# EI-CoreBioinformatics/portcullis

Hardware: AMD Instinct MI355X
Metric: junc_reads_per_sec (higher is better)
Workload: dtype int32; 1 GPU; BASELINE configs[2]: synthetic 199999998 paired-end 150-bp reads, 25 contigs of GRCh38 lengths (3088286401 bp), 249999 junctions, orientation FR; reads_total=199999998, junctions_total=249999, contigs=25, reads_rank0=199999998, pairs_rank0=66692850

## Files before the change

### portcullis_amd/csrc/pjb_api.hip

```cpp
#include "pjb_host.hip.h"
#include "pjb_kernels.hip.h"
#include "pjb_chain.hip.h"
#include "pjb_flight.hip.h"

extern "C" {

namespace {
std::mutex g_host_mu;
std::map<void *, size_t> g_host_registered;
}
void *pjb_host_alloc(size_t bytes) {
    if (bytes >= ((size_t)8 << 20)) {
        const size_t huge = (size_t)2 << 20, len = (bytes + huge - 1) & ~(huge - 1);
        void *p = mmap(nullptr, len, PROT_READ | PROT_WRITE, MAP_PRIVATE | MAP_ANONYMOUS, -1, 0);
        if (p != MAP_FAILED) {
            (void)madvise(p, len, MADV_HUGEPAGE);
            const size_t nt = std::min<size_t>(4, len >> 24);
            auto touch = [&](size_t t) {
                const size_t per = ((len / std::max<size_t>(nt, 1)) + huge - 1) & ~(huge - 1), a = std::min(len, per * t), b = std::min(len, a + per);
                for (size_t o = a; o < b; o += 4096) ((volatile uint8_t *)p)[o] = 0;
            };
            if (nt <= 1) touch(0);
            else {
                std::vector<std::thread> th;
// ... 664 lines not shown
    return PJB_OK;
}

int pjb_reset_kernel_timing(pjb_ctx *c) {
    if (!c) return PJB_ERR_ARG;
    std::fill(c->kcount.begin(), c->kcount.end(), 0);
    std::fill(c->kms.begin(), c->kms.end(), 0.0);
    return PJB_OK;
}

int pjb_set_option(pjb_ctx *c, const char *name, int64_t value) {
    if (!c || !name) return PJB_ERR_ARG;
    if (c->n_fl) return fail(c, PJB_ERR_STATE, "set_option: target %d is still queued", c->fl[0].tid);
    const std::string n = name;
    if (n == "overlap") c->side_stream = value != 0;
    else if (n == "dense_ids") c->dense_ids = value != 0;
    else if (n == "extra_dense") c->extra_dense_only = value != 0;
    else if (n == "sort_floor") c->sort_floor = (u32)std::max<int64_t>(1, std::min<int64_t>(value, 1 << 30));
    else if (n == "window_skip") c->window_skip = value != 0;
    else if (n == "run_sort") c->run_sort = value != 0;
    else if (n == "run_window") {
        if (value < 0 || value > (int64_t)RUN_W) return fail(c, PJB_ERR_ARG, "set_option: run_window takes 0 (the default, %u) to %u", RUN_W, RUN_W);
        c->run_window = (u32)value;
    } else if (n == "pair_range") {
        int shift = -1;
        for (int k = 0; k <= PAIR_RANGE_SHIFT_MAX; k++)
            if (value == (int64_t)1 << k) shift = k;
        if (shift < 0) return fail(c, PJB_ERR_ARG, "set_option: pair_range takes 1, 2, 4, 8, 16 or 32 slices a range (the default: %d)", 1 << PAIR_RANGE_SHIFT_DEFAULT);
        c->pair_range_shift = shift;
    } else if (n == "grow_batch") {
        if (value < 0 || value > 32768) return fail(c, PJB_ERR_ARG, "set_option: grow_batch takes 0 (the default: what the pool holds) to 32768 trees");
        c->model.grow_batch = (u32)value;
    } else if (n == "knn_chunk") {
        if (value < 0 || value > (1 << 22)) return fail(c, PJB_ERR_ARG, "set_option: knn_chunk takes 0 (the default: sized to fill the chip) to %d base rows", 1 << 22);
        c->model.knn_chunk = (u32)value;
    } else if (n == "mem_limit") {
        if (value < 0) return fail(c, PJB_ERR_ARG, "set_option: mem_limit takes 0 (the default: no limit) or a number of bytes");
        std::lock_guard<std::mutex> lk(c->mem.mu);
        c->mem.limit = (size_t)value;
    } else if (n == "list_cap") c->list_cap_forced = (u32)std::max<int64_t>(0, std::min<int64_t>(value, 1 << 30));
    else return fail(c, PJB_ERR_ARG, "set_option: unknown option '%s'", name);
    return PJB_OK;
}

int pjb_memory_info(const pjb_ctx *c, pjb_memory *out) {
    if (!c || !out) return PJB_ERR_ARG;
// ... 39 lines not shown
```

### portcullis_amd/csrc/pjb_chain.hip.h

```cpp
#pragma once

constexpr unsigned K6_BLOCKS = 128;

static size_t rows_upper_bound(const pjb_ctx *c) {
    size_t n = c->rows_n;
    for (int k = 0; k < c->n_fl; k++)
        if (c->fl[k].queued) n += c->fl[k].lim.junc_limit;
    return n;
}

static void wait_flight(pjb_ctx *c, Flight &f) {
    if (f.queued) (void)hipEventSynchronize(c->sl[f.slot].ev_done);
}

static int rows_table_reserve(pjb_ctx *c, Flight &f, u32 JL) {
    size_t old = rows_upper_bound(c);
    if (old + JL <= c->rows_cap) return PJB_OK;
    for (int k = 0; k < c->n_fl; k++)
        if (c->fl[k].queued && &c->fl[k] != &f) wait_flight(c, c->fl[k]);
    int rc = rows_sync(c);
    if (rc) return rc;
    old = std::min(old, c->rows_cap);
    const size_t ncap = std::max<size_t>((old + JL) * 3 / 2, 1024);
    pjb_junction_row *nd = (pjb_junction_row *)dev_alloc(c, MEM_ROWS, ncap * sizeof(pjb_junction_row));
// ... 3 lines not shown
        HIP_TRY(c, hipStreamSynchronize(c->stream4));
    }
    if (c->rows_table) bury(c, c->rows_table);
    c->rows_table = nd;
    c->rows_cap = ncap;
    return PJB_OK;
}

struct Chain {
    pjb_ctx *c;
    Flight &f;
    CtlSlot &S;
    hipStream_t st, service;
    GroupTab GT;
    bool group, fast_codes, any_x, stage_events, xk1, dense_moved, entropy_forked;
    int n_members;
    int32_t ref_len;
    KeyFmt kf;
    u32 PL, JL, SL;
    u32 n_tiles, pair_blocks, range_blocks, slots_lim, n_slices_lim, gen_cap, pack_nn;
    int range_shift;
    size_t n_words;
    int64_t row_base, mirror_base;
    u32 rs_tiles, run_cap, ro_tiles, plan_tiles;
    bool run_route, first_hist_done;
    int sort_bits, n_pass, pass_bits[16], cur;
    RunOut ro;
    u64 *ro_total, *ro_key[2];
    u32 *run_dest, *ro_idx[2];
    u64 *d_err;
    ContigStats *d_cs;
    const u32 *d_P, *d_J, *d_slots;
    MemberStats *d_members;
    u32 *d_member_junc, *d_tile_lo, *d_gen_cnt;
    Pairs pr;
};

struct ChainScope {
    pjb_ctx *c;
    hipStream_t stream = c->stream;
    Buf *scan_tiles = c->scan_tiles;
    int pool = c->cur_pool;
    ~ChainScope() {
        c->stream = stream;
        c->scan_tiles = scan_tiles;
        c->cur_pool = pool;
    }
};

#define STAGE_EVENT(k)                                                     \
    do {                                                                   \
        if (ch.stage_events) HIP_TRY(c, hipEventRecord(S.ev[k], ch.st));   \
// ... 41 lines not shown
        all_codes = all_codes && g.codes != nullptr;
        ch.any_x = ch.any_x || g.has_x;
    }
    ch.fast_codes = all_codes && !ch.any_x;
    ch.kf = lim.kf;
    const u32 PL = ch.PL = lim.pair_limit, JL = ch.JL = lim.junc_limit;
    ch.SL = lim.sort_limit && lim.sort_limit < JL ? lim.sort_limit : JL;
    bool ahead = false;
    for (int k = 0; k < c->n_fl; k++) ahead |= c->fl[k].queued && &c->fl[k] != &f;
    ch.row_base = ahead ? -1 : (int64_t)c->rows_n;
    ch.mirror_base = ahead ? -1 : (int64_t)c->mirror_rows;
    ch.pair_blocks = std::max<u32>(1, (PL + 255) / 256);
    ch.gen_cap = lim.list_cap ? lim.list_cap : (c->list_cap_forced ? c->list_cap_forced : gen_list_cap(PL));
    ch.pack_nn = (u64)ch.n_tiles * K1_TILE < (1ull << 28) ? 1u : 0u;
    ch.range_shift = c->pair_range_shift;
    ch.slots_lim = frag_slots_limit(JL, PL, ch.range_shift);
    ch.range_blocks = std::max<u32>(1, (frag_ranges(PL, ch.range_shift) + 3) / 4);
    ch.n_slices_lim = (PL + 63) / 64 + 1;
    ch.n_words = ((size_t)std::max(ch.ref_len, 1) + 63) / 64;
    ch.stage_events = c->ktime && c->ktime_only.empty();
    ch.xk1 = c->extra && !c->extra_dense_only && !ch.group && !f.x_k1 && !f.x_pre;
    ch.rs_tiles = std::max<u32>(1, (PL + RS_TILE - 1) / RS_TILE);
    ch.run_route = lim.dense && lim.run_sort;
    ch.run_cap = (u32)std::min<u64>((u64)PL / 8 + 64ull * ch.rs_tiles, 0xfff00000ull);
    ch.ro_tiles = (ch.run_cap + RS_TILE - 1) / RS_TILE;
    if (ch.run_route) {
        ch.ro.cap = ch.run_cap;
        ch.ro.window = c->run_window ? std::min<u32>(c->run_window, RUN_W) : RUN_W;
        ch.ro.tile_bits = std::max(1, bits_of((uint64_t)ch.rs_tiles));
    }
    ch.sort_bits = lim.dense ? std::max(1, bits_of((uint64_t)ch.SL)) + (ch.run_route ? ch.ro.tile_bits : 0) : ch.kf.total_bits;
    ch.plan_tiles = ch.run_route ? ch.ro_tiles : ch.rs_tiles;
    ch.first_hist_done = lim.dense && !ch.run_route;
    ch.n_pass = std::max(1, (ch.sort_bits + c->radix_max_bits - 1) / c->radix_max_bits);
    for (int p = 0; p < ch.n_pass; p++) ch.pass_bits[p] = ch.sort_bits / ch.n_pass + (p < ch.sort_bits % ch.n_pass ? 1 : 0);
    return PJB_OK;
}

static RunOut run_carve(Chain &ch, int &rc) {
    pjb_ctx *c = ch.c;
    CtlSlot &S = ch.S;
    RunOut ro = ch.ro;
    auto al = [](size_t b) { return (b + 255) & ~(size_t)255; };
    const u32 rs_tiles = ch.rs_tiles, run_cap = ch.run_cap;
    const size_t slack = (size_t)run_cap + RS_TILE;
    const size_t at_tf = 256, at_tn = at_tf + al((size_t)rs_tiles * 4), at_key = at_tn + al((size_t)rs_tiles * 4), at_cnt = at_key + al(slack * 8),
                 at_dest = at_cnt + al((size_t)run_cap * 4), at_k0 = at_dest + al((size_t)run_cap * 4), at_k1 = at_k0 + al(slack * 8),
                 at_i0 = at_k1 + al(slack * 8), at_i1 = at_i0 + al(slack * 4), at_end = at_i1 + al(slack * 4);
    if ((rc = ensure(c, S.runs, at_end))) return ro;
    uint8_t *b = (uint8_t *)S.runs.p;
    ro.n_runs = (u32 *)b;
    ch.ro_total = (u64 *)(b + 8);
    ro.tile_first = (u32 *)(b + at_tf);
    ro.tile_n = (u32 *)(b + at_tn);
    ro.key = (u64 *)(b + at_key);
    ro.cnt = (u32 *)(b + at_cnt);
    ch.run_dest = (u32 *)(b + at_dest);
    ch.ro_key[0] = (u64 *)(b + at_k0);
    ch.ro_key[1] = (u64 *)(b + at_k1);
    ch.ro_idx[0] = (u32 *)(b + at_i0);
    ch.ro_idx[1] = (u32 *)(b + at_i1);
    return ro;
}

static int chain_room(Chain &ch) {
    pjb_ctx *c = ch.c;
    Flight &f = ch.f;
    CtlSlot &S = ch.S;
    const std::vector<DevBatch> &batches = f.batches;
    const u32 PL = ch.PL, JL = ch.JL, n_tiles = ch.n_tiles;
    const size_t n_words = ch.n_words, N = (size_t)f.n_reads;
    const u32 plan_tiles = ch.plan_tiles;
    const int dbits = ch.pass_bits[0];
    const bool dense = f.lim.dense;
    int rc;
    if (batches.size() + 2 > S.batches_pinned_cap) {
        if (S.batches_pinned) (void)hipHostFree(S.batches_pinned);
        S.batches_pinned = nullptr;
        S.batches_pinned_cap = 0;
        const size_t cap = std::max<size_t>(batches.size() * 2 + 2, 16);
        HIP_TRY(c, hipHostMalloc((void **)&S.batches_pinned, cap * sizeof(DevBatch), hipHostMallocDefault));
        S.batches_pinned_cap = cap;
    }
    memcpy(S.batches_pinned, batches.data(), batches.size() * sizeof(DevBatch));
    const struct { Buf *b; size_t bytes; bool whole; } once[] = {
        {&S.scan_parts, sizeof(ScanPart) * K1S_BLOCKS, false},
        {&c->b_cursor, sizeof(RowCursor), false},
        {&S.members, GROUP_MAX * sizeof(MemberStats) + GROUP_MAX * 4 + (GROUP_MAX + 1) * 4, true},
    };
    for (const auto &o : once) {
        if (o.b->p) continue;
        if ((rc = ensure(c, *o.b, o.bytes))) return rc;
        HIP_TRY(c, hipMemset(o.b->p, 0, o.whole ? o.b->cap : o.bytes));
        HIP_TRY(c, hipStreamSynchronize(nullptr));
    }
    const void *was[3] = {S.bitmap.p, S.ends.p, S.pagecnt.p};
// ... 19 lines not shown
        {&S.jidbam, ((size_t)PL + RS_TILE) * 4},
        {&S.g, (size_t)PL * 4 + 16, c->extra},
        {&S.seg, ((size_t)PL + 1) * 4},
        {&S.runfirst, ((size_t)PL + 1) * 4},
        {&S.runstart, ((size_t)PL + 1) * 4},
        {&S.ent, (size_t)PL * 8 + 16},
        {&S.genlist, (size_t)ch.gen_cap * GEN_SHARDS * 8 * 3},
        {&S.gencount, GEN_SHARDS * GEN_CNT_STRIDE * 4},
        {&S.frag, (size_t)ch.slots_lim * F_WORDS * 4},
        {&S.fragj, (size_t)ch.slots_lim * 4},
        {&S.acc, (size_t)JL * F_WORDS * 4 + 16},
        {&S.ancl, (size_t)JL * 4 + 16},
        {&S.ancr, (size_t)JL * 4 + 16},
        {&S.jkey, (size_t)JL * 8 + 16},
        {&S.rows, (size_t)JL * sizeof(pjb_junction_row) + 16},
        {&S.entsum, (size_t)JL * 8 + 16},
        {&S.bitmap, n_words * 8 + 16, dense},
        {&S.wrank, n_words * 4 + 16, dense},
        {&S.pagecnt, ((n_words >> KD_PAGE_SHIFT) + 1) * 4 + 16, dense},
        {&S.pagerank, ((n_words >> KD_PAGE_SHIFT) + 1) * 4 + 16, dense},
        {&S.ends, (size_t)JL * DENSE_ENDS * 4 + 32, dense},
        {&S.firstid, (size_t)JL * 4 + 16, dense},
        {&S.masks, (size_t)ch.n_slices_lim * 8 * 2 + (size_t)ch.n_slices_lim * 4, dense},
        {&S.hist, (size_t)plan_tiles * (1u << dbits) * 4},
        {&S.hist_scan, (size_t)plan_tiles * (1u << dbits) * 4},
        {&S.bintotal, (size_t)4 << dbits},
        {&S.hist_part, (size_t)((plan_tiles + RSP_TILES - 1) / RSP_TILES) * (1u << dbits) * 4},
        {&S.x_q, N + 16, ch.xk1},
        {&S.x_spos, N * 4 + 16, ch.xk1},
        {&S.x_send, N * 4 + 16, ch.xk1},
        {&S.x_zlist, (size_t)X_ZCAP * 8, ch.xk1},
        {&S.x_scnt, X_SCNT_BYTES, ch.xk1},
    };
    for (const auto &r : room)
        if (r.on && (rc = ensure(c, *r.b, r.bytes))) return rc;
    ch.dense_moved = was[0] != S.bitmap.p || was[1] != S.ends.p || was[2] != S.pagecnt.p;
    if (ch.run_route) {
        ch.ro = run_carve(ch, rc);
        if (rc) return rc;
    }
    if ((rc = rows_table_reserve(c, f, JL))) return rc;
    if (!S.pub) {
        HIP_TRY(c, hipHostMalloc((void **)&S.pub, PUB_BYTES, hipHostMallocMapped | hipHostMallocPortable));
        void *dp = nullptr;
        if (hipHostGetDevicePointer(&dp, S.pub, 0) != hipSuccess || !dp) return fail(c, PJB_ERR_HIP, "hipHostGetDevicePointer(control block) failed");
        S.pub_dev = (uint8_t *)dp;
    }
    ch.d_members = (MemberStats *)S.members.p;
    ch.d_member_junc = (u32 *)(ch.d_members + GROUP_MAX);
    ch.d_tile_lo = ch.d_member_junc + GROUP_MAX;
// ... 128 lines not shown
    return PJB_OK;
}

static int chain_k2d(Chain &ch) {
    pjb_ctx *c = ch.c;
    Flight &f = ch.f;
    CtlSlot &S = ch.S;
    if (!f.lim.dense) return PJB_OK;
    const KeyFmt kf = ch.kf;
    const u32 JL = ch.JL;
    const size_t n_words = ch.n_words;
    int rc;
    const u32 cand_blocks = std::min<u32>(ch.pair_blocks, 1024u);
    const u64 *okey = (const u64 *)ch.pr.key;
    u64 *cand = (u64 *)S.key[1].p;
    const u32 n_pages = (u32)((n_words + ((size_t)1 << KD_PAGE_SHIFT) - 1) >> KD_PAGE_SHIFT);
    if ((rc = run_scan(c, "kd_rank", ArrU32Fn{(const u32 *)S.pagecnt.p}, ExclusiveU32Sink{(u32 *)S.pagerank.p}, (u64)n_pages, (u64 *)S.total.p)))
        return rc;
    LAUNCH(c, "kd_rank_pages", kd_rank_pages, dim3((n_pages + 3) / 4), dim3(256), (const u64 *)S.bitmap.p, (const u32 *)S.pagecnt.p, (const u32 *)S.pagerank.p,
           (u32 *)S.wrank.p, n_pages, (u32)n_words);
    u32 *cand_rank = (u32 *)S.idx[1].p;
    LAUNCH(c, "kd_ends", kd_ends, dim3(cand_blocks), dim3(256), (const u64 *)cand, kf, (const u64 *)S.bitmap.p, (const u32 *)S.wrank.p, JL,
           (u32 *)S.ends.p, cand_rank, ch.d_cs);
    if ((rc = run_scan(c, "kd_first", EndsCountFn{(const u32 *)S.ends.p}, FirstIdSink{(u32 *)S.firstid.p, (int32_t *)S.ancl.p, (int32_t *)S.ancr.p},
                       (u64)JL, (u64 *)S.total.p)))
        return rc;
    LAUNCH(c, "kd_table", kd_table, dim3(cand_blocks), dim3(256), (const u64 *)cand, (const u64 *)S.ent.p, (const u32 *)cand_rank, kf, JL,
           (const u32 *)S.ends.p, (const u32 *)S.firstid.p, (const u64 *)S.total.p, (u64 *)S.jkey.p, (int32_t *)S.ancl.p, (int32_t *)S.ancr.p, ch.d_cs,
           (const u32 *)ch.d_gen_cnt, ch.gen_cap, ch.SL, ch.ro.n_runs, ch.range_shift);
    LAUNCH(c, "kd_assign", kd_assign, dim3(ch.rs_tiles), dim3(256), okey, ch.d_P, kf, (const u64 *)S.bitmap.p, (const u32 *)S.wrank.p,
           (const u32 *)S.ends.p, (const u32 *)S.firstid.p, JL, (const u64 *)S.total.p, (u32 *)S.jidbam.p, (u32 *)S.acc.p, (const u64 *)S.jkey.p,
           (const int32_t *)S.ancl.p, (const int32_t *)S.ancr.p, ch.d_err, ch.d_cs, ch.run_route ? 0 : ch.pass_bits[0], (u32 *)S.hist.p, ch.ro);
    if ((rc = chain_fork(ch, S.ev_fork, S.ev_join, f.forked, chain_k4b))) return rc;
    LAUNCH(c, "kd_reset", kd_reset, dim3(cand_blocks), dim3(256), (const u64 *)cand, (const u32 *)cand_rank, kf, JL, (const ContigStats *)ch.d_cs,
           (u64 *)S.bitmap.p, (u32 *)S.ends.p, (u32 *)S.pagecnt.p);
    S.dense_at_rest = true;
    return PJB_OK;
}

static const char *const rs_names[4] = {"rs_hist", "rs_panel_sums", "rs_panel_scan", "rs_scatter"};
static const char *const ro_names[6] = {"ro_hist", "ro_panel_sums", "ro_panel_scan", "ro_scatter", "ro_offsets", "rs_place"};

template <typename K>
static int sort_pass(Chain &ch, const void *kin_v, void *kout_v, const u32 *vin, u32 *vout, int shift, int bits, const u32 *d_n, u32 tiles,
                     const char *const *names) {
    pjb_ctx *c = ch.c;
    CtlSlot &S = ch.S;
    const K *kin = (const K *)kin_v;
    K *kout = (K *)kout_v;
    if (!(shift == 0 && ch.first_hist_done))
        LAUNCH(c, names[0], rs_hist<K>, dim3(tiles), dim3(256), kin, d_n, shift, bits, (u32 *)S.hist.p, tiles);
    {
        const u32 nb = 1u << bits, n_panels = (tiles + RSP_TILES - 1) / RSP_TILES;
        LAUNCH(c, names[1], rs_panel_sums, dim3(n_panels, (nb + 255) / 256), dim3(256), (const u32 *)S.hist.p, tiles, nb, (u32 *)S.hist_part.p);
        LAUNCH(c, names[2], rs_panel_scan, dim3(n_panels, (nb + 255) / 256), dim3(256), (const u32 *)S.hist.p, (const u32 *)S.hist_part.p, tiles, nb,
               (u32 *)S.hist_scan.p, (u32 *)S.bintotal.p);
    }
#define RS_SCATTER(B)                                                                                                                          \
    LAUNCH_LDS(c, names[3], (rs_scatter<B, K>), dim3(tiles), dim3(256), rs_scatter_lds_bytes(bits, sizeof(K)), kin, vin, kout, vout, d_n, \
               shift, bits, (const u32 *)S.hist_scan.p, (const u32 *)S.bintotal.p, tiles)
    switch (bits) {
    case 9: RS_SCATTER(9); break;
    case 10: RS_SCATTER(10); break;
    case 11: RS_SCATTER(11); break;
    default: RS_SCATTER(0); break;
    }
#undef RS_SCATTER
    return PJB_OK;
}

static int chain_sort(Chain &ch) {
    pjb_ctx *c = ch.c;
    Flight &f = ch.f;
    CtlSlot &S = ch.S;
    const RunOut &ro = ch.ro;
    int rc = PJB_OK, cur = 0, shift = 0;
    for (int p = 0; p < ch.n_pass; p++) {
        const int bits = ch.pass_bits[p];
        if (bits <= 0) break;
        if (ch.run_route) {
            rc = sort_pass<u64>(ch, p == 0 ? (const void *)ro.key : (const void *)ch.ro_key[cur], ch.ro_key[cur ^ 1], p == 0 ? nullptr : (const u32 *)ch.ro_idx[cur],
                                ch.ro_idx[cur ^ 1], shift, bits, (const u32 *)ro.n_runs, ch.ro_tiles, ro_names);
        } else {
            const u32 *vin = p == 0 ? nullptr : (const u32 *)S.idx[cur].p;
            u32 *vout = (u32 *)S.idx[cur ^ 1].p;
            if (f.lim.dense) rc = sort_pass<u32>(ch, p == 0 ? S.jidbam.p : S.key[cur].p, S.key[cur ^ 1].p, vin, vout, shift, bits, ch.d_P, ch.rs_tiles, rs_names);
            else rc = sort_pass<u64>(ch, p == 0 ? S.okey.p : S.key[cur].p, S.key[cur ^ 1].p, vin, vout, shift, bits, ch.d_P, ch.rs_tiles, rs_names);
        }
        if (rc) return rc;
        cur ^= 1;
        shift += bits;
    }
    f.n_pass = ch.n_pass;
    if (ch.run_route) {
        const u32 *order = ch.ro_idx[cur];
        if ((rc = run_scan(c, ro_names[4], RunCountFn{(const u32 *)ro.cnt, order}, RunDestSink{ch.run_dest, order}, (u64)ch.run_cap, ch.ro_total, (const u32 *)ro.n_runs)))
            return rc;
        cur = 1;
        LAUNCH(c, ro_names[5], rs_place, dim3(ch.rs_tiles), dim3(256), (const u32 *)S.jidbam.p, ch.d_P, (const u64 *)ro.key, (const u32 *)ch.run_dest,
               (const u32 *)ro.tile_first, (const u32 *)ro.tile_n, ch.run_cap, ro.tile_bits, (u32 *)S.key[cur].p, (u32 *)S.idx[cur].p);
        f.n_pass = 1;
    }
    ch.cur = cur;
    f.sidx = (const u32 *)S.idx[cur].p;
    f.jid_sorted = f.lim.dense ? (const u32 *)S.key[cur].p : (const u32 *)S.jid.p;
    STAGE_EVENT(2);
    return PJB_OK;
}

static int chain_entropy(Chain &ch) {
    pjb_ctx *c = ch.c;
    CtlSlot &S = ch.S;
    LAUNCH(c, "k5_entropy_sum", k5_entropy_sum, dim3(std::max<u32>(1, (ch.JL + 15) / 16)), dim3(256), (const u32 *)S.seg.p, (const u32 *)S.runfirst.p,
           (const u32 *)S.runstart.p, ch.d_J, (double *)S.entsum.p);
    return PJB_OK;
}

#ifdef PJB_DEBUG_LAUNCH
static void debug_sort_check(Chain &ch) {
    Flight &f = ch.f;
    CtlSlot &S = ch.S;
    const int cur = ch.cur;
// ... 137 lines not shown
```

### portcullis_amd/csrc/pjb_device.hip.h

```cpp
#pragma once

#include <hip/hip_runtime.h>
#include <stdint.h>

#include "../../include/portcullis_amd.h"

namespace pjb {

typedef unsigned long long u64;
typedef unsigned int u32;

struct DevBatch {
    const int32_t *pos;
    const uint16_t *flag;
    const uint8_t *mapq;
    const uint8_t *xs;
    const int32_t *l_qseq;
    const int32_t *mtid;
    const int32_t *mpos;
    const uint32_t *cig_off;
    const uint32_t *cigar;
    const uint32_t *seq_off;
    const uint8_t *seq4;
    const u64 *name_hash;
// ... 606 lines not shown
constexpr int RS_ITEMS = 16;
constexpr int RS_TILE = 256 * RS_ITEMS;
constexpr int RS_MAX_BITS = 12;
constexpr int RS_MAX_BINS = 1 << RS_MAX_BITS;
constexpr int KDA_TILE = RS_TILE;
static_assert(RS_MAX_BINS <= 4096, "kd_assign counts the sort's first digit tile by tile");

__device__ __forceinline__ void wave_hist_add(u32 *h, u32 d, bool valid) {
    u64 rem = __ballot(valid);
    const int lane = lane_id();
#pragma unroll
    for (int it = 0; it < 2; it++) {
        if (rem == 0) return;
        const int first = __ffsll((long long)rem) - 1;
        const u32 d0 = __shfl(d, first, 64);
        const u64 m = __ballot(valid && d == d0) & rem;
        if (lane == first) atomicAdd(&h[d0], (u32)__popcll(m));
        rem &= ~m;
    }
    if ((rem >> lane) & 1ull) atomicAdd(&h[d], 1u);
}

constexpr u32 RUN_W = 2048;
struct RunOut {
    u64 *key;
    u32 *cnt;
    u32 *tile_first;
    u32 *tile_n;
    u32 *n_runs;
    u32 cap;
    u32 window;
    int tile_bits;
};

enum {
    F_N = 0, F_R1P, F_R1N, F_R2P, F_R2N, F_MS, F_XSP, F_XSN, F_UM, F_BPP, F_PPP, F_REL, F_DIST,
    F_MAXMINANC, F_UP, F_DOWN, F_MAXMMES, F_MAXMINMATCH,
    F_FIRSTMIS,
    F_PAD19,
    F_MISM_LO, F_MISM_HI,
    F_JAD0,
    F_WORDS = 48
};
__device__ __forceinline__ void acc_rest_state(u32 *acc, u64 n_junc) {
    const u64 n = n_junc * F_WORDS, step = (u64)gridDim.x * blockDim.x;
    for (u64 t = (u64)blockIdx.x * blockDim.x + threadIdx.x; t < n; t += step) acc[t] = (t % F_WORDS) == F_FIRSTMIS ? 100000000u : 0u;
}

}
```

### portcullis_amd/csrc/pjb_host.hip.h

```cpp
#pragma once
#include "pjb_device.hip.h"
#include "pjb_extra_types.hip.h"
#include "pjb_memory.hip.h"

#include <algorithm>
#include <sys/mman.h>
#include <thread>
#include <chrono>
#include <cstdarg>
#include <cstdio>
#include <cstdlib>
#include <cstring>
#include <map>
#include <memory>
#include <mutex>
#include <string>
#include <thread>
#include <unordered_map>
#include <vector>

using namespace pjb;


inline thread_local std::string g_create_error;
// ... 220 lines not shown
    int last_slot = 0;
    int inflate_lanes = 512 * 64;
    bool side_stream = true;
    bool dense_ids = true;
    u32 junc_seen = 0;
    int lbits_seen = 18;
    size_t rows_n = 0, rows_cap = 0;
    size_t rows_pinned_cap = 0;
    std::vector<void *> graveyard;
    std::mutex grave_mu;
    size_t last_rows_n = 0;
    uint8_t *mirror = nullptr;
    size_t mirror_cap = 0;
    int64_t *mirror_hdr = nullptr;
    size_t mirror_rows = 0;
    int64_t mirror_acc[5] = {0, 0, 0, INT32_MAX, 0};
    pjb_timing timing;
    int radix_max_bits = 11;
    double junc_per_read = 0;
    u32 sort_floor = 1u << 16;
    bool window_skip = true;
    bool run_sort = true;
    u32 run_window = 0;
    int pair_range_shift = PAIR_RANGE_SHIFT_DEFAULT;
    u32 list_cap_forced = 0;
    bool k1_serial = true;
    hipEvent_t last_k1_ev = nullptr;
    int k1s_blocks_forced = 0;
    bool ktime = false;
    std::vector<std::string> knames;
    std::vector<int64_t> kcount;
    std::vector<double> kms;
    std::vector<std::string> ktime_only;
    Buf *scan_tiles = nullptr;
    Buf b_scan_tiles;
    Buf b_inf_comp, b_inf_out, b_inf_blocks, b_inf_status, b_inf_scratch, b_inf_bitmap;
    Buf b_dfl_in, b_dfl_sym, b_dfl_slots, b_dfl_size, b_dfl_off, b_dfl_packed;
    Buf b_bam_seg, b_bam_rec, b_bam_ctl;
    struct IndexState *index = nullptr;
    bool extra = false;
    std::vector<ExtraContig> xc;
    std::map<int32_t, std::pair<u64 *, u32>> filter_keys;
    Buf f_pos, f_cigoff, f_cigar, f_codes;
    ModelState model;
    Buf x_pos, x_endx, x_q, x_prefq, x_ce, x_bound, x_de, x_dropped, x_zlist, x_cnt, x_tabk, x_tabc, x_rs, x_re, x_rr, x_tileoff;
    Buf x_xrall, x_tab;
// ... 551 lines not shown
```

### portcullis_amd/csrc/pjb_k2_sort.hip.h

```cpp
#pragma once

#include "pjb_device.hip.h"

namespace pjb {


template <typename K>
__global__ __launch_bounds__(256) void rs_hist(const K *keys, const u32 *np, int shift, int bits, u32 *hist, u32 n_tiles) {
    __shared__ u32 h[RS_MAX_BINS];
    const u32 n = *np;
    const u32 nb = 1u << bits;
    for (u32 d = threadIdx.x; d < nb; d += 256) h[d] = 0;
    __syncthreads();
    const u32 base = blockIdx.x * RS_TILE;
    const u32 mask = nb - 1;
    K kk[RS_ITEMS];
#pragma unroll
    for (int k = 0; k < RS_ITEMS; k++) {
        const u32 i = base + k * 256 + threadIdx.x;
        kk[k] = i < n ? keys[i] : (K)0;
    }
#pragma unroll
    for (int k = 0; k < RS_ITEMS; k++) {
        const u32 i = base + k * 256 + threadIdx.x;
// ... 167 lines not shown
    u32 digp[RS_ITEMS / 2];
#pragma unroll
    for (int r = 0; r < RS_ITEMS; r++) {
        const u32 j = r * 256 + threadIdx.x;
        const K kk = j < cnt ? kbuf[j] : (K)0;
        const u32 d = (u32)(kk >> shift) & mask;
        digp[r >> 1] = (r & 1) ? (digp[r >> 1] | (d << 16)) : d;
        if (j < cnt) kout[delta[d] + j] = kk;
    }
    __syncthreads();
#pragma unroll
    for (int r = 0; r < RS_ITEMS; r++) {
        const u32 i = base + r * 64 + lane;
        if (i < n) ibuf[(rkp[r >> 1] >> ((r & 1) * 16)) & 0xffffu] = val[r];
    }
    __syncthreads();
#pragma unroll
    for (int r = 0; r < RS_ITEMS; r++) {
        const u32 j = r * 256 + threadIdx.x;
        if (j < cnt) vout[delta[(digp[r >> 1] >> ((r & 1) * 16)) & 0xffffu] + j] = ibuf[j];
    }
}

struct RunCountFn {
    const u32 *cnt, *order;
    __device__ u64 operator()(u64 i) const { return cnt[order[i]]; }
};
struct RunDestSink {
    u32 *dest;
    const u32 *order;
    __device__ void operator()(u64 i, u64, u64 ex) const { dest[order[i]] = (u32)ex; }
};
__global__ __launch_bounds__(256) void rs_place(const u32 *jid_bam, const u32 *np, const u64 *run_key, const u32 *run_dest, const u32 *tile_first,
                                                const u32 *tile_n, u32 run_cap, int tile_bits, u32 *kout, u32 *vout) {
    __shared__ u32 s_dest[RUN_W];
    __shared__ unsigned short s_wcnt[4][RUN_W];
    const u32 n = *np;
    const u32 tile = blockIdx.x;
    if ((u64)tile * RS_TILE >= n) return;
    for (u32 d = threadIdx.x; d < 2 * RUN_W; d += 256) ((u32 *)&s_wcnt[0][0])[d] = 0;
    const u32 tf = tile_first[tile], tn = tf < run_cap ? min(tile_n[tile], min(RUN_W, run_cap - tf)) : 0u;
    for (u32 e = threadIdx.x; e < tn; e += 256) s_dest[(u32)(run_key[tf + e] >> tile_bits) & (RUN_W - 1u)] = run_dest[tf + e];
    const int w = __builtin_amdgcn_readfirstlane(threadIdx.x >> 6), lane = lane_id();
    unsigned short *wc = s_wcnt[w];
    const u32 base = tile * RS_TILE + w * (RS_TILE / 4);
    const u64 lt = (1ull << lane) - 1;
    u32 id[RS_ITEMS];
    u32 rkp[RS_ITEMS / 2];
    const u32 *kp = jid_bam + base;
#pragma unroll
    for (int r = 0; r < RS_ITEMS; r++) id[r] = kp[r * 64 + lane];
    __syncthreads();
#pragma unroll
    for (int r = 0; r < RS_ITEMS; r++) {
        const bool valid = base + r * 64 + lane < n;
// ... 35 lines not shown
```

### portcullis_amd/csrc/pjb_k2d_ids.hip.h

```cpp
#pragma once

#include "pjb_device.hip.h"

namespace pjb {

constexpr int DENSE_ENDS = 8;
constexpr u32 DENSE_EMPTY = 0xffffffffu;

__device__ __forceinline__ u32 start_rank(const u64 *bitmap, const u32 *wrank, int32_t start) {
    const u32 w = (u32)start >> 6;
    return wrank[w] + (u32)__popcll(bitmap[w] & ((1ull << (start & 63)) - 1ull));
}
struct PopcFn {
    const u64 *words;
    __device__ u64 operator()(u64 i) const { return (u64)__popcll(words[i]); }
};
__global__ __launch_bounds__(256) void kd_ends(const u64 *cand, KeyFmt kf, const u64 *bitmap, const u32 *wrank, u32 junc_limit, u32 *ends,
                                               u32 *cand_rank, ContigStats *cs) {
    const u32 n = cs->n_cand;
    for (u32 p = blockIdx.x * 256 + threadIdx.x; p < n; p += gridDim.x * 256) {
        int32_t s, e;
        unpack_key(kf, cand[p], s, e);
        const u32 rs = start_rank(bitmap, wrank, s);
        cand_rank[p] = rs;
// ... 31 lines not shown
        const u32 rs = cand_rank[p];
        if (rs < junc_limit) {
            uint4 *q = reinterpret_cast<uint4 *>(ends + (size_t)rs * DENSE_ENDS);
            q[0] = q[1] = make_uint4(DENSE_EMPTY, DENSE_EMPTY, DENSE_EMPTY, DENSE_EMPTY);
        }
    }
}
struct EndsCountFn {
    const u32 *ends;
    __device__ u64 operator()(u64 rs) const {
        const uint4 *q = reinterpret_cast<const uint4 *>(ends + rs * DENSE_ENDS);
        const uint4 a = q[0], b = q[1];
        return (u64)((a.x != DENSE_EMPTY) + (a.y != DENSE_EMPTY) + (a.z != DENSE_EMPTY) + (a.w != DENSE_EMPTY) + (b.x != DENSE_EMPTY) +
                     (b.y != DENSE_EMPTY) + (b.z != DENSE_EMPTY) + (b.w != DENSE_EMPTY));
    }
};
struct FirstIdSink {
    u32 *first_id;
    int32_t *anc_l, *anc_r;
    __device__ void operator()(u64 i, u64, u64 ex) const {
        first_id[i] = (u32)ex;
        anc_l[i] = INT32_MAX;
        anc_r[i] = INT32_MIN;
    }
};
__device__ __forceinline__ u32 ends_below(const u32 *ends, u32 rs, u32 ue) {
    const uint4 *q = reinterpret_cast<const uint4 *>(ends + (size_t)rs * DENSE_ENDS);
    const uint4 a = q[0], b = q[1];
    return (a.x < ue) + (a.y < ue) + (a.z < ue) + (a.w < ue) + (b.x < ue) + (b.y < ue) + (b.z < ue) + (b.w < ue);
}

__global__ __launch_bounds__(256) void kd_table(const u64 *cand, const u64 *cand_anc, const u32 *cand_rank, KeyFmt kf, u32 junc_limit, const u32 *ends,
                                                const u32 *first_id, const u64 *total, u64 *jkey, int32_t *anc_l, int32_t *anc_r, ContigStats *cs,
                                                const u32 *gen_cnt, u32 gen_cap, u32 sort_limit, u32 *n_runs, int range_shift) {
    const u32 p = blockIdx.x * 256 + threadIdx.x;
    if (blockIdx.x == 0) {
        static_assert(GEN_SHARDS == 256, "a shard per thread of the first block");
        const u32 over = lists_over(gen_cnt, threadIdx.x, gen_cap);
        if (over) atomicMax(&cs->list_need, over);
        if (__syncthreads_or((int)over) && threadIdx.x == 0) cs->overflow |= OVF_LISTS;
    }
    if (p == 0) {
        if (n_runs) *n_runs = 0;
        const u64 J = *total;
        u32 ovf = cs->overflow;
        if (cs->P != 0 && (J > (u64)junc_limit || J > (u64)sort_limit)) {
// ... 170 lines not shown
        u32 c[8], nz = 0;
#pragma unroll
        for (int k = 0; k < 8; k++) {
            const u32 o = threadIdx.x * 8u + (u32)k;
            c[k] = o < span ? s_h[(lo + o) & (RUN_W - 1u)] : 0u;
            nz += c[k] != 0u;
        }
        u32 tot;
        u32 at = block_escan_256<u32>(nz, s_rscan, &tot);
        if (threadIdx.x == 0) {
            u32 b = atomicAdd(ro.n_runs, tot);
            if (b > ro.cap || tot > ro.cap - b) {
                atomicSub(ro.n_runs, tot);
                b = 0xffffffffu;
                runs_close_chain(cs_chk);
            }
            s_run[2] = b;
            ro.tile_first[blockIdx.x] = b == 0xffffffffu ? 0u : b;
            ro.tile_n[blockIdx.x] = b == 0xffffffffu ? 0u : tot;
        }
        __syncthreads();
        const u32 first = s_run[2];
        if (first == 0xffffffffu) return;
        at += first;
#pragma unroll
        for (int k = 0; k < 8; k++)
            if (c[k]) {
                ro.key[at] = ((u64)(lo + threadIdx.x * 8u + (u32)k) << ro.tile_bits) | (u64)blockIdx.x;
                ro.cnt[at] = c[k];
                at++;
            }
    }
}

}
```

Baseline: 31.34 billion reads/s.

## Replace multi-pass radix sort of run keys with per-id bucketing and ranking

The run-route path no longer radix-sorts run keys by (id, tile). Each run now takes a ticket from a per-id atomic counter when it is emitted, which also accumulates the pair counts. A scan over ids then gives bucket bases, rp_bucket scatters runs into their id segments, and rp_rank computes each run's destination by summing the counts of earlier tiles within the segment. This removes several histogram, scan and scatter passes over the runs, but adds global atomics in the emit kernel and a quadratic scan for ids whose runs span many tiles, bounded by a fan limit that closes the chain when exceeded.

```diff
diff --git a/portcullis_amd/csrc/pjb_api.hip b/portcullis_amd/csrc/pjb_api.hip
--- a/portcullis_amd/csrc/pjb_api.hip
+++ b/portcullis_amd/csrc/pjb_api.hip
@@ -710,6 +710,9 @@
     else if (n == "run_window") {
         if (value < 0 || value > (int64_t)RUN_W) return fail(c, PJB_ERR_ARG, "set_option: run_window takes 0 (the default, %u) to %u", RUN_W, RUN_W);
         c->run_window = (u32)value;
+    } else if (n == "run_fan") {
+        if (value < 0 || value > (int64_t)1 << 20) return fail(c, PJB_ERR_ARG, "set_option: run_fan takes 0 (the default, %u) to %d", RUN_FAN, 1 << 20);
+        c->run_fan = (u32)value;
     } else if (n == "pair_range") {
         int shift = -1;
         for (int k = 0; k <= PAIR_RANGE_SHIFT_MAX; k++)
diff --git a/portcullis_amd/csrc/pjb_chain.hip.h b/portcullis_amd/csrc/pjb_chain.hip.h
--- a/portcullis_amd/csrc/pjb_chain.hip.h
+++ b/portcullis_amd/csrc/pjb_chain.hip.h
@@ -49,12 +49,12 @@
     int range_shift;
     size_t n_words;
     int64_t row_base, mirror_base;
-    u32 rs_tiles, run_cap, ro_tiles, plan_tiles;
+    u32 rs_tiles, run_cap;
     bool run_route, first_hist_done;
     int sort_bits, n_pass, pass_bits[16], cur;
     RunOut ro;
-    u64 *ro_total, *ro_key[2];
-    u32 *run_dest, *ro_idx[2];
+    u64 *ro_total, *id_base, *seg_tc, *seg_ir;
+    u32 *run_dest;
     u64 *d_err;
     ContigStats *d_cs;
     const u32 *d_P, *d_J, *d_slots;
@@ -142,15 +142,14 @@
     ch.xk1 = c->extra && !c->extra_dense_only && !ch.group && !f.x_k1 && !f.x_pre;
     ch.rs_tiles = std::max<u32>(1, (PL + RS_TILE - 1) / RS_TILE);
     ch.run_route = lim.dense && lim.run_sort;
-    ch.run_cap = (u32)std::min<u64>((u64)PL / 8 + 64ull * ch.rs_tiles, 0xfff00000ull);
-    ch.ro_tiles = (ch.run_cap + RS_TILE - 1) / RS_TILE;
+    ch.run_cap = run_list_cap(PL, ch.rs_tiles);
     if (ch.run_route) {
         ch.ro.cap = ch.run_cap;
         ch.ro.window = c->run_window ? std::min<u32>(c->run_window, RUN_W) : RUN_W;
+        ch.ro.fan = c->run_fan ? c->run_fan : RUN_FAN;
         ch.ro.tile_bits = std::max(1, bits_of((uint64_t)ch.rs_tiles));
     }
-    ch.sort_bits = lim.dense ? std::max(1, bits_of((uint64_t)ch.SL)) + (ch.run_route ? ch.ro.tile_bits : 0) : ch.kf.total_bits;
-    ch.plan_tiles = ch.run_route ? ch.ro_tiles : ch.rs_tiles;
+    ch.sort_bits = lim.dense ? std::max(1, bits_of((uint64_t)ch.SL)) : ch.kf.total_bits;
     ch.first_hist_done = lim.dense && !ch.run_route;
     ch.n_pass = std::max(1, (ch.sort_bits + c->radix_max_bits - 1) / c->radix_max_bits);
     for (int p = 0; p < ch.n_pass; p++) ch.pass_bits[p] = ch.sort_bits / ch.n_pass + (p < ch.sort_bits % ch.n_pass ? 1 : 0);
@@ -161,25 +160,21 @@
     pjb_ctx *c = ch.c;
     CtlSlot &S = ch.S;
     RunOut ro = ch.ro;
-    auto al = [](size_t b) { return (b + 255) & ~(size_t)255; };
-    const u32 rs_tiles = ch.rs_tiles, run_cap = ch.run_cap;
-    const size_t slack = (size_t)run_cap + RS_TILE;
-    const size_t at_tf = 256, at_tn = at_tf + al((size_t)rs_tiles * 4), at_key = at_tn + al((size_t)rs_tiles * 4), at_cnt = at_key + al(slack * 8),
-                 at_dest = at_cnt + al((size_t)run_cap * 4), at_k0 = at_dest + al((size_t)run_cap * 4), at_k1 = at_k0 + al(slack * 8),
-                 at_i0 = at_k1 + al(slack * 8), at_i1 = at_i0 + al(slack * 4), at_end = at_i1 + al(slack * 4);
-    if ((rc = ensure(c, S.runs, at_end))) return ro;
+    const RunRoom at = run_room(ch.rs_tiles, ch.run_cap, ch.JL);
+    if ((rc = ensure(c, S.runs, at.end))) return ro;
     uint8_t *b = (uint8_t *)S.runs.p;
     ro.n_runs = (u32 *)b;
     ch.ro_total = (u64 *)(b + 8);
-    ro.tile_first = (u32 *)(b + at_tf);
-    ro.tile_n = (u32 *)(b + at_tn);
-    ro.key = (u64 *)(b + at_key);
-    ro.cnt = (u32 *)(b + at_cnt);
-    ch.run_dest = (u32 *)(b + at_dest);
-    ch.ro_key[0] = (u64 *)(b + at_k0);
-    ch.ro_key[1] = (u64 *)(b + at_k1);
-    ch.ro_idx[0] = (u32 *)(b + at_i0);
-    ch.ro_idx[1] = (u32 *)(b + at_i1);
+    ro.tile_first = (u32 *)(b + at.tile_first);
+    ro.tile_n = (u32 *)(b + at.tile_n);
+    ro.key = (u64 *)(b + at.key);
+    ro.cnt = (u32 *)(b + at.cnt);
+    ro.tick = (u32 *)(b + at.tick);
+    ro.id_cnt = (u64 *)(b + at.id_cnt);
+    ch.run_dest = (u32 *)(b + at.dest);
+    ch.seg_tc = (u64 *)(b + at.seg_tc);
+    ch.seg_ir = (u64 *)(b + at.seg_ir);
+    ch.id_base = (u64 *)(b + at.id_base);
     return ro;
 }
 
@@ -190,8 +185,9 @@
     const std::vector<DevBatch> &batches = f.batches;
     const u32 PL = ch.PL, JL = ch.JL, n_tiles = ch.n_tiles;
     const size_t n_words = ch.n_words, N = (size_t)f.n_reads;
-    const u32 plan_tiles = ch.plan_tiles;
+    const u32 plan_tiles = ch.rs_tiles;
     const int dbits = ch.pass_bits[0];
+    const bool radix = !ch.run_route;
     const bool dense = f.lim.dense;
     int rc;
     if (batches.size() + 2 > S.batches_pinned_cap) {
@@ -257,10 +253,10 @@
         {&S.ends, (size_t)JL * DENSE_ENDS * 4 + 32, dense},
         {&S.firstid, (size_t)JL * 4 + 16, dense},
         {&S.masks, (size_t)ch.n_slices_lim * 8 * 2 + (size_t)ch.n_slices_lim * 4, dense},
-        {&S.hist, (size_t)plan_tiles * (1u << dbits) * 4},
-        {&S.hist_scan, (size_t)plan_tiles * (1u << dbits) * 4},
-        {&S.bintotal, (size_t)4 << dbits},
-        {&S.hist_part, (size_t)((plan_tiles + RSP_TILES - 1) / RSP_TILES) * (1u << dbits) * 4},
+        {&S.hist, (size_t)plan_tiles * (1u << dbits) * 4, radix},
+        {&S.hist_scan, (size_t)plan_tiles * (1u << dbits) * 4, radix},
+        {&S.bintotal, (size_t)4 << dbits, radix},
+        {&S.hist_part, (size_t)((plan_tiles + RSP_TILES - 1) / RSP_TILES) * (1u << dbits) * 4, radix},
         {&S.x_q, N + 16, ch.xk1},
         {&S.x_spos, N * 4 + 16, ch.xk1},
         {&S.x_send, N * 4 + 16, ch.xk1},
@@ -435,8 +431,10 @@
     u32 *cand_rank = (u32 *)S.idx[1].p;
     LAUNCH(c, "kd_ends", kd_ends, dim3(cand_blocks), dim3(256), (const u64 *)cand, kf, (const u64 *)S.bitmap.p, (const u32 *)S.wrank.p, JL,
            (u32 *)S.ends.p, cand_rank, ch.d_cs);
-    if ((rc = run_scan(c, "kd_first", EndsCountFn{(const u32 *)S.ends.p}, FirstIdSink{(u32 *)S.firstid.p, (int32_t *)S.ancl.p, (int32_t *)S.ancr.p},
-                       (u64)JL, (u64 *)S.total.p)))
+    if ((rc = ch.run_route ? run_scan(c, "kd_first", EndsCountFn{(const u32 *)S.ends.p},
+                                      FirstIdRunSink{(u32 *)S.firstid.p, (int32_t *)S.ancl.p, (int32_t *)S.ancr.p, ch.ro.id_cnt}, (u64)JL, (u64 *)S.total.p)
+                           : run_scan(c, "kd_first", EndsCountFn{(const u32 *)S.ends.p}, FirstIdSink{(u32 *)S.firstid.p, (int32_t *)S.ancl.p, (int32_t *)S.ancr.p},
+                                      (u64)JL, (u64 *)S.total.p)))
         return rc;
     LAUNCH(c, "kd_table", kd_table, dim3(cand_blocks), dim3(256), (const u64 *)cand, (const u64 *)S.ent.p, (const u32 *)cand_rank, kf, JL,
            (const u32 *)S.ends.p, (const u32 *)S.firstid.p, (const u64 *)S.total.p, (u64 *)S.jkey.p, (int32_t *)S.ancl.p, (int32_t *)S.ancr.p, ch.d_cs,
@@ -452,7 +450,7 @@
 }
 
 static const char *const rs_names[4] = {"rs_hist", "rs_panel_sums", "rs_panel_scan", "rs_scatter"};
-static const char *const ro_names[6] = {"ro_hist", "ro_panel_sums", "ro_panel_scan", "ro_scatter", "ro_offsets", "rs_place"};
+static const char *const rp_names[4] = {"rp_ids", "rp_bucket", "rp_rank", "rs_place"};
 
 template <typename K>
 static int sort_pass(Chain &ch, const void *kin_v, void *kout_v, const u32 *vin, u32 *vout, int shift, int bits, const u32 *d_n, u32 tiles,
@@ -488,29 +486,27 @@
     CtlSlot &S = ch.S;
     const RunOut &ro = ch.ro;
     int rc = PJB_OK, cur = 0, shift = 0;
-    for (int p = 0; p < ch.n_pass; p++) {
+    for (int p = 0; p < ch.n_pass && !ch.run_route; p++) {
         const int bits = ch.pass_bits[p];
         if (bits <= 0) break;
-        if (ch.run_route) {
-            rc = sort_pass<u64>(ch, p == 0 ? (const void *)ro.key : (const void *)ch.ro_key[cur], ch.ro_key[cur ^ 1], p == 0 ? nullptr : (const u32 *)ch.ro_idx[cur],
-                                ch.ro_idx[cur ^ 1], shift, bits, (const u32 *)ro.n_runs, ch.ro_tiles, ro_names);
-        } else {
-            const u32 *vin = p == 0 ? nullptr : (const u32 *)S.idx[cur].p;
-            u32 *vout = (u32 *)S.idx[cur ^ 1].p;
-            if (f.lim.dense) rc = sort_pass<u32>(ch, p == 0 ? S.jidbam.p : S.key[cur].p, S.key[cur ^ 1].p, vin, vout, shift, bits, ch.d_P, ch.rs_tiles, rs_names);
-            else rc = sort_pass<u64>(ch, p == 0 ? S.okey.p : S.key[cur].p, S.key[cur ^ 1].p, vin, vout, shift, bits, ch.d_P, ch.rs_tiles, rs_names);
-        }
+        const u32 *vin = p == 0 ? nullptr : (const u32 *)S.idx[cur].p;
+        u32 *vout = (u32 *)S.idx[cur ^ 1].p;
+        if (f.lim.dense) rc = sort_pass<u32>(ch, p == 0 ? S.jidbam.p : S.key[cur].p, S.key[cur ^ 1].p, vin, vout, shift, bits, ch.d_P, ch.rs_tiles, rs_names);
+        else rc = sort_pass<u64>(ch, p == 0 ? S.okey.p : S.key[cur].p, S.key[cur ^ 1].p, vin, vout, shift, bits, ch.d_P, ch.rs_tiles, rs_names);
         if (rc) return rc;
         cur ^= 1;
         shift += bits;
     }
     f.n_pass = ch.n_pass;
     if (ch.run_route) {
-        const u32 *order = ch.ro_idx[cur];
-        if ((rc = run_scan(c, ro_names[4], RunCountFn{(const u32 *)ro.cnt, order}, RunDestSink{ch.run_dest, order}, (u64)ch.run_cap, ch.ro_total, (const u32 *)ro.n_runs)))
-            return rc;
+        const u32 rp_blocks = std::max<u32>(1, std::min<u32>((ch.run_cap + 255) / 256, RP_BLOCKS));
+        if ((rc = run_scan(c, rp_names[0], IdCountFn{(const u64 *)ro.id_cnt}, IdBaseSink{ch.id_base}, (u64)ch.JL, ch.ro_total, ch.d_J))) return rc;
+        LAUNCH(c, rp_names[1], rp_bucket, dim3(rp_blocks), dim3(256), ch.d_P, ch.d_J, ch.JL, (const u64 *)ro.key, (const u32 *)ro.cnt, (const u32 *)ro.tick,
+               (const u32 *)ro.n_runs, ch.run_cap, ro.tile_bits, (const u64 *)ch.id_base, ch.seg_tc, ch.seg_ir);
+        LAUNCH(c, rp_names[2], rp_rank, dim3(rp_blocks), dim3(256), ch.d_P, ch.d_J, ch.JL, (const u32 *)ro.n_runs, ch.run_cap, (const u64 *)ch.id_base,
+               (const u64 *)ch.seg_tc, (const u64 *)ch.seg_ir, ch.run_dest);
         cur = 1;
-        LAUNCH(c, ro_names[5], rs_place, dim3(ch.rs_tiles), dim3(256), (const u32 *)S.jidbam.p, ch.d_P, (const u64 *)ro.key, (const u32 *)ch.run_dest,
+        LAUNCH(c, rp_names[3], rs_place, dim3(ch.rs_tiles), dim3(256), (const u32 *)S.jidbam.p, ch.d_P, (const u64 *)ro.key, (const u32 *)ch.run_dest,
                (const u32 *)ro.tile_first, (const u32 *)ro.tile_n, ch.run_cap, ro.tile_bits, (u32 *)S.key[cur].p, (u32 *)S.idx[cur].p);
         f.n_pass = 1;
     }
diff --git a/portcullis_amd/csrc/pjb_device.hip.h b/portcullis_amd/csrc/pjb_device.hip.h
--- a/portcullis_amd/csrc/pjb_device.hip.h
+++ b/portcullis_amd/csrc/pjb_device.hip.h
@@ -652,16 +652,43 @@
 }
 
 constexpr u32 RUN_W = 2048;
+constexpr u32 RUN_FAN = 2048;
 struct RunOut {
     u64 *key;
     u32 *cnt;
+    u32 *tick;
     u32 *tile_first;
     u32 *tile_n;
     u32 *n_runs;
+    u64 *id_cnt;
     u32 cap;
     u32 window;
+    u32 fan;
     int tile_bits;
 };
+__host__ __device__ constexpr u32 run_list_cap(u32 pair_limit, u32 tiles) {
+    const u64 want = (u64)pair_limit / 8 + 64ull * tiles;
+    return (u32)(want < 0xfff00000ull ? want : 0xfff00000ull);
+}
+struct RunRoom {
+    size_t tile_first, tile_n, key, cnt, tick, dest, seg_tc, seg_ir, id_cnt, id_base, end;
+};
+inline RunRoom run_room(u32 tiles, u32 cap, u32 junc_limit) {
+    auto al = [](size_t b) { return (b + 255) & ~(size_t)255; };
+    RunRoom r;
+    r.tile_first = 256;
+    r.tile_n = r.tile_first + al((size_t)tiles * 4);
+    r.key = r.tile_n + al((size_t)tiles * 4);
+    r.cnt = r.key + al((size_t)cap * 8);
+    r.tick = r.cnt + al((size_t)cap * 4);
+    r.dest = r.tick + al((size_t)cap * 4);
+    r.seg_tc = r.dest + al((size_t)cap * 4);
+    r.seg_ir = r.seg_tc + al((size_t)cap * 8);
+    r.id_cnt = r.seg_ir + al((size_t)cap * 8);
+    r.id_base = r.id_cnt + al((size_t)junc_limit * 8);
+    r.end = r.id_base + al(((size_t)junc_limit + 1) * 8);
+    return r;
+}
 
 enum {
     F_N = 0, F_R1P, F_R1N, F_R2P, F_R2N, F_MS, F_XSP, F_XSN, F_UM, F_BPP, F_PPP, F_REL, F_DIST,
diff --git a/portcullis_amd/csrc/pjb_host.hip.h b/portcullis_amd/csrc/pjb_host.hip.h
--- a/portcullis_amd/csrc/pjb_host.hip.h
+++ b/portcullis_amd/csrc/pjb_host.hip.h
@@ -266,6 +266,7 @@
     bool window_skip = true;
     bool run_sort = true;
     u32 run_window = 0;
+    u32 run_fan = 0;
     int pair_range_shift = PAIR_RANGE_SHIFT_DEFAULT;
     u32 list_cap_forced = 0;
     bool k1_serial = true;
diff --git a/portcullis_amd/csrc/pjb_k2_sort.hip.h b/portcullis_amd/csrc/pjb_k2_sort.hip.h
--- a/portcullis_amd/csrc/pjb_k2_sort.hip.h
+++ b/portcullis_amd/csrc/pjb_k2_sort.hip.h
@@ -213,15 +213,53 @@
     }
 }
 
-struct RunCountFn {
-    const u32 *cnt, *order;
-    __device__ u64 operator()(u64 i) const { return cnt[order[i]]; }
+struct IdCountFn {
+    const u64 *id_cnt;
+    __device__ u64 operator()(u64 i) const { return id_cnt[i]; }
 };
-struct RunDestSink {
-    u32 *dest;
-    const u32 *order;
-    __device__ void operator()(u64 i, u64, u64 ex) const { dest[order[i]] = (u32)ex; }
+struct IdBaseSink {
+    u64 *id_base;
+    __device__ void operator()(u64 i, u64, u64 ex) const { id_base[i] = ex; }
 };
+constexpr u32 RP_BLOCKS = 1024;
+__global__ __launch_bounds__(256) void rp_bucket(const u32 *np, const u32 *nj, u32 junc_limit, const u64 *run_key, const u32 *run_cnt, const u32 *run_tick,
+                                                 const u32 *n_runs, u32 run_cap, int tile_bits, const u64 *id_base, u64 *seg_tc, u64 *seg_ir) {
+    if (*np == 0) return;
+    const u32 n = min(*n_runs, run_cap), J = min(*nj, junc_limit);
+    for (u32 r = blockIdx.x * 256 + threadIdx.x; r < n; r += gridDim.x * 256) {
+        const u64 key = run_key[r];
+        const u32 id = (u32)(key >> tile_bits), tile = (u32)(key & ((1ull << tile_bits) - 1ull));
+        if (id >= J) continue;
+        const u32 slot = (u32)(id_base[id] >> 32) + run_tick[r];
+        if (slot >= n) continue;
+        seg_tc[slot] = ((u64)tile << 32) | run_cnt[r];
+        seg_ir[slot] = ((u64)id << 32) | r;
+    }
+}
+__global__ __launch_bounds__(256) void rp_rank(const u32 *np, const u32 *nj, u32 junc_limit, const u32 *n_runs, u32 run_cap, const u64 *id_base,
+                                               const u64 *seg_tc, const u64 *seg_ir, u32 *run_dest) {
+    if (*np == 0) return;
+    const u32 n = min(*n_runs, run_cap), J = min(*nj, junc_limit);
+    for (u32 s = blockIdx.x * 256 + threadIdx.x; s < n; s += gridDim.x * 256) {
+        const u64 ir = seg_ir[s];
+        const u32 id = (u32)(ir >> 32), r = (u32)ir;
+        if (id >= J || r >= n) continue;
+        const u64 b = id_base[id];
+        const u32 a = (u32)(b >> 32), e = id + 1 < J ? min((u32)(id_base[id + 1] >> 32), n) : n;
+        u32 dest = (u32)b;
+        if (e - a > 1 && e > a) {
+            const u32 tile = (u32)(seg_tc[s] >> 32);
+            for (u32 q = a; q < e; q += 8) {
+                u64 v[8];
+#pragma unroll
+                for (u32 j = 0; j < 8; j++) v[j] = q + j < e ? seg_tc[q + j] : ~0ull;
+#pragma unroll
+                for (u32 j = 0; j < 8; j++) dest += (u32)(v[j] >> 32) < tile ? (u32)v[j] : 0u;
+            }
+        }
+        run_dest[r] = dest;
+    }
+}
 __global__ __launch_bounds__(256) void rs_place(const u32 *jid_bam, const u32 *np, const u64 *run_key, const u32 *run_dest, const u32 *tile_first,
                                                 const u32 *tile_n, u32 run_cap, int tile_bits, u32 *kout, u32 *vout) {
     __shared__ u32 s_dest[RUN_W];
diff --git a/portcullis_amd/csrc/pjb_k2d_ids.hip.h b/portcullis_amd/csrc/pjb_k2d_ids.hip.h
--- a/portcullis_amd/csrc/pjb_k2d_ids.hip.h
+++ b/portcullis_amd/csrc/pjb_k2d_ids.hip.h
@@ -77,6 +77,17 @@
         first_id[i] = (u32)ex;
         anc_l[i] = INT32_MAX;
         anc_r[i] = INT32_MIN;
+    }
+};
+struct FirstIdRunSink {
+    u32 *first_id;
+    int32_t *anc_l, *anc_r;
+    u64 *id_cnt;
+    __device__ void operator()(u64 i, u64, u64 ex) const {
+        first_id[i] = (u32)ex;
+        anc_l[i] = INT32_MAX;
+        anc_r[i] = INT32_MIN;
+        id_cnt[i] = 0;
     }
 };
 __device__ __forceinline__ u32 ends_below(const u32 *ends, u32 rs, u32 ue) {
@@ -293,15 +304,23 @@
         __syncthreads();
         const u32 first = s_run[2];
         if (first == 0xffffffffu) return;
-        at += first;
+        static_assert(2 * RUN_W <= 4096 && KDA_TILE <= 0xffff, "the compacted runs (id - lo) << 16 | pairs fit s_h's upper half");
+        u32 *s_ent = s_h + RUN_W;
 #pragma unroll
         for (int k = 0; k < 8; k++)
-            if (c[k]) {
-                ro.key[at] = ((u64)(lo + threadIdx.x * 8u + (u32)k) << ro.tile_bits) | (u64)blockIdx.x;
-                ro.cnt[at] = c[k];
-                at++;
-            }
-    }
-}
-
-}
+            if (c[k]) s_ent[at++] = ((threadIdx.x * 8u + (u32)k) << 16) | c[k];
+        __syncthreads();
+        bool wide = false;
+        for (u32 j = threadIdx.x; j < tot; j += 256) {
+            const u32 e = s_ent[j], id = lo + (e >> 16), pairs = e & 0xffffu;
+            ro.key[first + j] = ((u64)id << ro.tile_bits) | (u64)blockIdx.x;
+            ro.cnt[first + j] = pairs;
+            const u32 t = id < junc_limit ? (u32)(atomicAdd(&ro.id_cnt[id], (1ull << 32) | (u64)pairs) >> 32) : ro.fan;
+            ro.tick[first + j] = t;
+            wide = wide || t >= ro.fan;
+        }
+        if (wide) runs_close_chain(cs_chk);
+    }
+}
+
+}
```

Measured after the change: 31.48 billion reads/s (median of 6 runs). No clear change (+0.5%).
